# rcelha/rio-rs

Measured on NVIDIA H100. Metric: placements/sec, higher is better.
Workload: dtype u32

## Files before the change

rio_rs_b200/csrc/engine.cu:

```cuda
#include "../../include/rio_cuda.h"
#include "../../include/rio_cuda_dev.h"
#include "kernels.cuh"
#include "k_ranked.cuh"
#include "k_affinity_ranked.cuh"
#include "k_affinity_spread.cuh"
#include "k_affinity_set.cuh"
#include "k_affinity_bounded.cuh"
#include "k_set_bounded_affinity.cuh"
#include "k_set_churn.cuh"
#include "k_set_commit.cuh"
#include "k_bounded_weighted.cuh"
#include "k_changes.cuh"
#include "k_ranked_changes.cuh"
#include "k_spread.cuh"
#include "k_spread_changes.cuh"
#include "spec.cuh"
#include "trie_table.hpp"

#include <dlfcn.h>

#include <algorithm>
#include <atomic>
#include <chrono>
#include <cstdio>
// ... 231 lines not shown
    return h->h_scalars[which];
}
void check_device_error(rio_placement *h) {
    uint32_t e = 0;
    CUDA_TRY(cudaMemcpyAsync(&e, h->d_error(), 4, cudaMemcpyDeviceToHost, h->stream));
    CUDA_TRY(cudaStreamSynchronize(h->stream));
    if (e) { CUDA_TRY(cudaMemsetAsync(h->d_error(), 0, 4, h->stream)); throw RioError{RIO_ERR_UNKNOWN, "directory table overflow (internal sizing error)"}; }
}

bool address_malformed(const std::string &a) {
    size_t c = a.find(':');
    return c == std::string::npos || c == 0 || c + 1 >= a.size();
}

uint32_t intern_node(rio_placement *h, const std::string &addr) {
    auto it = h->node_index.find(addr);
    if (it != h->node_index.end()) return it->second;
    REQUIRE(h->nodes.size() < 0xFFFFFFF0u, "too many nodes");
    NodeInfo ni;
    ni.addr = addr;
    ni.seed = mix64(fnv1a64(addr.data(), addr.size()));
    ni.seed2 = mix64(ni.seed ^ kSaltNode2);
    ni.malformed = address_malformed(addr);
    uint32_t idx = (uint32_t)h->nodes.size();
    h->nodes.push_back(std::move(ni));
    h->node_index.emplace(addr, idx);
    h->tab_dirty = true;
    return idx;
}

void build_tab(rio_placement *h, TabBufs &tb, const std::vector<uint8_t> *closed) {
    const uint32_t n_total = (uint32_t)h->nodes.size();
    struct Ent { uint32_t invw, idx; };
    std::vector<Ent> live;
    auto is_closed = [&](uint32_t j) { return closed && j < closed->size() && (*closed)[j]; };
    for (uint32_t j = 0; j < n_total; j++) {
        const NodeInfo &ni = h->nodes[j];
        if (!ni.live()) continue;
        if (is_closed(j)) continue;
        live.push_back(Ent{inv_weight(ni.weight), j});
    }
    {
        std::vector<uint32_t> classes_seen;
        bool few = true;
        for (const Ent &e : live) {
            if (std::find(classes_seen.begin(), classes_seen.end(), e.invw) != classes_seen.end()) continue;
            if (classes_seen.size() == 64) { few = false; break; }
            classes_seen.push_back(e.invw);
        }
        if (few) {
            std::sort(classes_seen.begin(), classes_seen.end());
            std::vector<uint32_t> start(classes_seen.size() + 1, 0);
            auto cls = [&](uint32_t invw) { return (size_t)(std::lower_bound(classes_seen.begin(), classes_seen.end(), invw) - classes_seen.begin()); };
            for (const Ent &e : live) start[cls(e.invw) + 1]++;
            for (size_t c = 0; c < classes_seen.size(); c++) start[c + 1] += start[c];
            std::vector<Ent> grouped(live.size());
            for (const Ent &e : live) grouped[start[cls(e.invw)]++] = e;
            live.swap(grouped);
        } else {
            std::sort(live.begin(), live.end(), [](const Ent &a, const Ent &b) { return a.invw != b.invw ? a.invw < b.invw : a.idx < b.idx; });
        }
    }
    std::vector<NodeRec> recs(live.size() ? live.size() : 1);
    std::vector<ClassRec> classes;
    for (size_t q = 0; q < live.size(); q++) {
        const NodeInfo &ni = h->nodes[live[q].idx];
        recs[q] = NodeRec{(uint32_t)ni.seed, live[q].idx, (uint32_t)(ni.seed >> 32) | 1u, (uint32_t)ni.seed2};
        if (q == 0 || live[q].invw != live[q - 1].invw || (h->dev_table_flags & RIO_DEV_SPLIT_CLASSES)) classes.push_back(ClassRec{(uint32_t)q, live[q].invw});
    }
    const uint32_t n_classes = (uint32_t)classes.size();
    classes.push_back(ClassRec{(uint32_t)live.size(), 0});
    classes.push_back(ClassRec{(uint32_t)live.size(), 0});
    std::vector<uint4> by_idx(n_total ? n_total : 1);
    for (uint32_t j = 0; j < n_total; j++) {
        const NodeInfo &ni = h->nodes[j];
        const bool lv = ni.live() && !is_closed(j);
        by_idx[j] = make_uint4((uint32_t)ni.seed, lv ? inv_weight(ni.weight) : 0u, (uint32_t)(ni.seed >> 32) | 1u, (uint32_t)ni.seed2);
    }
    std::vector<TrieMember> members;
    members.reserve(live.size());
    for (const Ent &e : live) members.push_back(TrieMember{h->nodes[e.idx].seed, e.idx, h->nodes[e.idx].weight});
    const TrieBlob blob = build_trie_blob(members, h->trie_bits);
    const uint32_t bits = blob.bits, nb = 1u << bits, blob_bytes = blob.blob_bytes;
    std::vector<uint8_t> state(n_total ? n_total : 1, 0);
    std::vector<uint32_t> livef(n_total ? n_total : 1, 0);
    for (uint32_t j = 0; j < n_total; j++) {
        const NodeInfo &ni = h->nodes[j];
        state[j] = ((ni.active && !ni.malformed) ? kNodeLive : 0) | (ni.malformed ? kNodeMalformed : 0);
        livef[j] = (ni.live() && !is_closed(j)) ? 1u : 0u;
    }

    auto al = [](size_t v) { return (v + 255) & ~(size_t)255; };
    const size_t o_recs = 0, o_classes = al(o_recs + recs.size() * sizeof(NodeRec)), o_byidx = al(o_classes + classes.size() * sizeof(ClassRec)),
                 o_trie = al(o_byidx + by_idx.size() * sizeof(uint4)), o_state = al(o_trie + blob_bytes), o_live = al(o_state + state.size()),
                 total = al(o_live + livef.size() * 4);
    cudaStream_t st = h->stream;
    if (tb.upload_pending) { CUDA_TRY(cudaStreamSynchronize(st)); tb.upload_pending = false; }
    if (h->aux_stream) CUDA_TRY(cudaStreamSynchronize(h->aux_stream));
    if (total > tb.stage_cap) {
        if (tb.stage) CUDA_TRY(cudaFreeHost(tb.stage));
        tb.stage = nullptr; tb.stage_cap = 0;
        CUDA_TRY(cudaMallocHost(reinterpret_cast<void **>(&tb.stage), total * 2));
        tb.stage_cap = total * 2;
    }
    memcpy(tb.stage + o_recs, recs.data(), recs.size() * sizeof(NodeRec));
    memcpy(tb.stage + o_classes, classes.data(), classes.size() * sizeof(ClassRec));
    memcpy(tb.stage + o_byidx, by_idx.data(), by_idx.size() * sizeof(uint4));
    memcpy(tb.stage + o_trie, blob.words.data(), blob_bytes);
    memcpy(tb.stage + o_state, state.data(), state.size());
    memcpy(tb.stage + o_live, livef.data(), livef.size() * 4);
    tb.dev.ensure(total, st);
    CUDA_TRY(cudaMemcpyAsync(tb.dev.p, tb.stage, total, cudaMemcpyHostToDevice, st));
    tb.upload_pending = true;
    unsigned char *d = tb.dev.as<unsigned char>();
    tb.trie = TrieDev{d + o_trie, blob_bytes, blob.off_crec, bits, blob.n_chain, {}};
    for (uint32_t i = 1; i < 8 && i < nb; i++) tb.trie.top[i] = blob.words[i];
    tb.tab.recs = reinterpret_cast<const NodeRec *>(d + o_recs);
    tb.tab.classes = reinterpret_cast<const ClassRec *>(d + o_classes);
    tb.tab.by_idx = reinterpret_cast<const uint4 *>(d + o_byidx);
    tb.tab.n_live = (uint32_t)live.size();
    tb.tab.n_classes = n_classes;
    tb.tab.n_total = n_total;
    tb.state = d + o_state;
    tb.live = reinterpret_cast<const uint32_t *>(d + o_live);
}

uint64_t live_signature(const rio_placement *h) {
    uint64_t sig = kFnvBasis;
    for (uint32_t j = 0; j < (uint32_t)h->nodes.size(); j++)
        if (h->nodes[j].live()) sig = mix64(sig ^ (((uint64_t)j << 32) | h->nodes[j].weight));
    return sig;
}

void build_aff_operands(rio_placement *h, const std::vector<uint8_t> *closed, DevBuf &fc_buf, DevBuf &fg_buf, DevBuf &map_buf, uint32_t &n_live,
                        uint32_t &n_pad) {
    const uint32_t n_total = (uint32_t)h->nodes.size();
    cudaStream_t st = h->stream;
    auto is_closed = [&](uint32_t j) { return closed && j < closed->size() && (*closed)[j]; };
    std::vector<uint32_t> map;
    for (uint32_t j = 0; j < n_total; j++) if (h->nodes[j].live() && !is_closed(j)) map.push_back(j);
    const uint32_t nl = (uint32_t)map.size();
    const uint32_t pad = nl <= 64 ? 64 : (nl + 255) / 256 * 256;
    std::vector<float> fc((size_t)pad * 16, 0.f);
    for (uint32_t q = 0; q < nl; q++) if (h->nodes[map[q]].feat.size() == 16) std::copy(h->nodes[map[q]].feat.begin(), h->nodes[map[q]].feat.end(), fc.begin() + (size_t)q * 16);
    map.resize(pad, kNone);
    std::vector<float> fg(fc.size());
    for (uint32_t g8 = 0; g8 < pad / 8; g8++)
        for (uint32_t k4 = 0; k4 < 4; k4++)
            for (uint32_t r8 = 0; r8 < 8; r8++)
                std::copy_n(fc.begin() + ((size_t)g8 * 8 + r8) * 16 + k4 * 4, 4, fg.begin() + (((size_t)g8 * 4 + k4) * 8 + r8) * 4);
    fc_buf.ensure(fc.size() * 4, st);
    fg_buf.ensure(fg.size() * 4, st);
    CUDA_TRY(cudaMemcpyAsync(fg_buf.p, fg.data(), fg.size() * 4, cudaMemcpyHostToDevice, st));
    map_buf.ensure(map.size() * 4, st);
    CUDA_TRY(cudaMemcpyAsync(fc_buf.p, fc.data(), fc.size() * 4, cudaMemcpyHostToDevice, st));
    CUDA_TRY(cudaMemcpyAsync(map_buf.p, map.data(), map.size() * 4, cudaMemcpyHostToDevice, st));
    CUDA_TRY(cudaStreamSynchronize(st));
    n_live = nl; n_pad = pad;
}

void ensure_tab(rio_placement *h) {
    if (!h->tab_dirty) return;
    build_tab(h, h->tabs, nullptr);
    const uint32_t n_total = (uint32_t)h->nodes.size();
    cudaStream_t st = h->stream;
    h->tab_dirty = false;
    h->tab_version++;
    h->live_sig = live_signature(h);
    if (!h->K) return;
    std::vector<float> fnode((size_t)(n_total ? n_total : 1) * h->K, 0.f);
    for (uint32_t j = 0; j < n_total; j++) {
        const NodeInfo &ni = h->nodes[j];
        if (ni.feat.size() == h->K) std::copy(ni.feat.begin(), ni.feat.end(), fnode.begin() + (size_t)j * h->K);
    }
    h->d_fnode.ensure(fnode.size() * 4, st);
    CUDA_TRY(cudaMemcpyAsync(h->d_fnode.p, fnode.data(), fnode.size() * 4, cudaMemcpyHostToDevice, st));
    h->aff_live = h->aff_pad = 0;
    if (h->K == 16) build_aff_operands(h, nullptr, h->d_fnode_c, h->d_fnode_g, h->d_nidx_map, h->aff_live, h->aff_pad);
    CUDA_TRY(cudaStreamSynchronize(st));
}

uint64_t pow2_at_least(uint64_t v) { uint64_t p = 1; while (p < v) p <<= 1; return p; }

void dir_alloc(rio_placement *h, uint64_t cap, DirDev &out) {
    void *p = nullptr;
    CUDA_TRY(cudaMallocAsync(&p, cap * sizeof(DirSlot), h->stream));
    out.slots = reinterpret_cast<DirSlot *>(p);
    out.mask = cap - 1;
    uint32_t lg = 0; while ((1ull << lg) < cap) lg++;
    out.shift = 64 - lg;
    launch_dir_init(h->L(), out.slots, cap);
}

void reconcile_dir_keys(rio_placement *h) {
    h->dir_keys = read_scalar(h, S_NEWKEYS);
    h->dir_keys_pending = 0;
}

// ... 2478 lines not shown
```

rio_rs_b200/csrc/k_trie.cu:

```cuda
#include "kernels.cuh"
#include "spec.cuh"
#include "bounded_tail.cuh"

#include <cstdlib>

namespace rio {

namespace {

constexpr int kTrieThreads = 256;
constexpr uint32_t kMaxLevels = 16;

__constant__ uint32_t c_lvl_s0[kMaxLevels];
__constant__ uint32_t c_lvl_m2[kMaxLevels];
__constant__ uint32_t c_lvl_h2[kMaxLevels];

__device__ __forceinline__ uint32_t smem_u32(const void *p) { return (uint32_t)__cvta_generic_to_shared(p); }

__device__ __forceinline__ void stage_blob_tma(void *smem_dst, const void *gsrc, uint32_t bytes, unsigned long long *bar) {
    if (threadIdx.x == 0) {
        asm volatile("mbarrier.init.shared::cta.b64 [%0], 1;" ::"r"(smem_u32(bar)) : "memory");
        asm volatile("fence.mbarrier_init.release.cluster;" ::: "memory");
    }
    __syncthreads();
    if (threadIdx.x == 0) {
        asm volatile("mbarrier.arrive.expect_tx.shared::cta.b64 _, [%0], %1;" ::"r"(smem_u32(bar)), "r"(bytes) : "memory");
        for (uint32_t off = 0; off < bytes; off += 32768u) {
            const uint32_t len = min(32768u, bytes - off);
            asm volatile("cp.async.bulk.shared::cluster.global.mbarrier::complete_tx::bytes [%0], [%1], %2, [%3];"
                         ::"r"(smem_u32(reinterpret_cast<unsigned char *>(smem_dst) + off)),
                           "l"(reinterpret_cast<const unsigned char *>(gsrc) + off), "r"(len), "r"(smem_u32(bar))
                         : "memory");
        }
    }
    uint32_t done = 0;
    while (!done) {
        asm volatile("{\n\t.reg .pred p;\n\tmbarrier.try_wait.parity.shared::cta.b64 p, [%1], %2;\n\tselp.u32 %0, 1, 0, p;\n\t}"
                     : "=r"(done) : "r"(smem_u32(bar)), "r"(0u) : "memory");
    }
}

__device__ __forceinline__ uint32_t walk_step(uint32_t off, uint32_t sel) {
    uint32_t r;
    asm("mad.lo.u32 %0, %1, 2, %2;" : "=r"(r) : "r"(off), "r"(sel));
    return r;
}

template <int BITS>
__device__ __forceinline__ uint32_t trie_leaf_index(ObjHash o, const uint32_t *__restrict__ tab32, uint32_t bits_rt) {
    uint32_t i = 1;
    if (BITS > 0) {
#pragma unroll
        for (int l = 0; l < BITS; l++) {
            const uint32_t u = contest_u(o, c_lvl_s0[l], c_lvl_m2[l], c_lvl_h2[l]);
            i = 2 * i + (u > tab32[i] ? 1u : 0u);
        }
    } else {
        for (uint32_t l = 0; l < bits_rt; l++) {
            const uint32_t u = contest_u(o, c_lvl_s0[l], c_lvl_m2[l], c_lvl_h2[l]);
            i = 2 * i + (u > tab32[i] ? 1u : 0u);
        }
    }
    return i;
}

__device__ __forceinline__ uint32_t trie_resolve_leaf(ObjHash o, uint32_t leaf, const unsigned char *__restrict__ blob) {
    if ((int32_t)leaf > -2) return leaf;
    uint32_t w = leaf;
    for (;;) {
        const unsigned char *p = blob + (w & 0x7FFFFFFFu);
        const uint4 r = *reinterpret_cast<const uint4 *>(p);
        const uint2 nn = *reinterpret_cast<const uint2 *>(p + 16);
        if (contest_u(o, r.x, r.y, r.z) <= r.w) return nn.x;
        if ((int32_t)nn.y >= 0) return nn.y;
        w = nn.y;
    }
}

struct TrieSmem {
    const uint32_t *tab32;
    const unsigned char *blob;
    uint32_t *hist;
};

template <bool SMEM>
__device__ __forceinline__ TrieSmem trie_stage(const TrieDev &t, uint32_t hist_bins) {
    extern __shared__ __align__(128) unsigned char smem_trie[];
    constexpr bool in_smem = SMEM;
    TrieSmem s;
    uint32_t off = 0;
    if (in_smem) {
        s.tab32 = reinterpret_cast<const uint32_t *>(smem_trie);
        s.blob = smem_trie;
        off = t.blob_bytes;
    } else {
        const unsigned char *g = reinterpret_cast<const unsigned char *>(t.blob);
        s.tab32 = reinterpret_cast<const uint32_t *>(g);
        s.blob = g;
    }
    s.hist = reinterpret_cast<uint32_t *>(smem_trie + off);
    for (uint32_t j = threadIdx.x; j < hist_bins; j += blockDim.x) s.hist[j] = 0;
    unsigned long long *bar = reinterpret_cast<unsigned long long *>(smem_trie + off + ((hist_bins * 4u + 15u) & ~15u));
    if (in_smem) stage_blob_tma(smem_trie, t.blob, t.blob_bytes, bar);
    else __syncthreads();
    return s;
}

template <int BITS, int OPT, int MODE, bool SMEM, int MINB = (SMEM ? 5 : 3)>
__global__ void __launch_bounds__(kTrieThreads, MINB)
k_assign_trie(const uint64_t *__restrict__ keys, uint64_t n, TrieDev t, uint32_t *__restrict__ out_idx, uint32_t *__restrict__ counters,
              uint32_t hist_bins, unsigned long long *__restrict__ moved, const __grid_constant__ BoundedTail tail) {
    static_assert(OPT % 2 == 0, "two objects per 128-bit load");
    constexpr bool in_smem = SMEM;
    constexpr int SEG = OPT / 2;
    const uint64_t tile_objs = (uint64_t)kTrieThreads * OPT;
    const uint64_t n_tiles = (n + tile_objs - 1) / tile_objs;
    unsigned long long n_moved = 0;
    ulonglong2 kk[SEG];
    auto load_tile = [&](uint64_t tile) {
        const uint64_t f0 = tile * tile_objs + 2 * threadIdx.x;
        if ((tile + 1) * tile_objs <= n) {
            const ulonglong2 *src = reinterpret_cast<const ulonglong2 *>(keys + f0);
#pragma unroll
            for (int g = 0; g < SEG; g++) kk[g] = __ldg(src + g * kTrieThreads);
            return;
        }
#pragma unroll
        for (int g = 0; g < SEG; g++) {
            const uint64_t f = f0 + (uint64_t)g * (2 * kTrieThreads);
            kk[g] = make_ulonglong2(0, 0);
            if (f + 1 < n) kk[g] = __ldg(reinterpret_cast<const ulonglong2 *>(keys + f));
            else if (f < n) kk[g].x = __ldg(keys + f);
        }
    };
    const TrieSmem s = trie_stage<SMEM>(t, hist_bins);
    asm volatile("griddepcontrol.launch_dependents;" ::: "memory");
    asm volatile("griddepcontrol.wait;" ::: "memory");
    if (blockIdx.x < n_tiles) load_tile(blockIdx.x);
    for (uint64_t tile = blockIdx.x; tile < n_tiles; tile += gridDim.x) {
        const uint64_t base = tile * tile_objs;
        const bool full_tile = base + tile_objs <= n;
        ObjHash o[OPT];
#pragma unroll
        for (int g = 0; g < SEG; g++) {
            o[2 * g] = obj_hash(kk[g].x);
            o[2 * g + 1] = obj_hash(kk[g].y);
        }
        if (tile + gridDim.x < n_tiles) load_tile(tile + gridDim.x);
        uint32_t leaf[OPT];
        if (in_smem) {
            const unsigned char *tb = reinterpret_cast<const unsigned char *>(s.tab32);
            uint32_t off[OPT];
#pragma unroll
            for (int k = 0; k < OPT; k++) off[k] = 4;
            if (BITS > 0) {
                constexpr int TOP = BITS >= 3 ? 3 : 0;
                if (TOP) {
#pragma unroll
                    for (int k = 0; k < OPT; k++) {
                        const bool c0 = contest_u(o[k], c_lvl_s0[0], c_lvl_m2[0], c_lvl_h2[0]) > t.top[1];
                        const bool c1 = contest_u(o[k], c_lvl_s0[1], c_lvl_m2[1], c_lvl_h2[1]) > (c0 ? t.top[3] : t.top[2]);
                        const uint32_t t2 = c0 ? (c1 ? t.top[7] : t.top[6]) : (c1 ? t.top[5] : t.top[4]);
                        const bool c2 = contest_u(o[k], c_lvl_s0[2], c_lvl_m2[2], c_lvl_h2[2]) > t2;
                        off[k] = 32u + (c0 ? 16u : 0u) + (c1 ? 8u : 0u) + (c2 ? 4u : 0u);
                    }
                }
#pragma unroll
                for (int l = TOP; l < BITS; l++) {
#pragma unroll
                    for (int k = 0; k < OPT; k++) {
                        const uint32_t u = contest_u(o[k], c_lvl_s0[l], c_lvl_m2[l], c_lvl_h2[l]);
                        const uint32_t thr = *reinterpret_cast<const uint32_t *>(tb + off[k]);
                        off[k] = walk_step(off[k], u > thr ? 4u : 0u);
                    }
                }
            } else {
                for (uint32_t l = 0; l < t.bits; l++) {
#pragma unroll
                    for (int k = 0; k < OPT; k++) {
                        const uint32_t u = contest_u(o[k], c_lvl_s0[l], c_lvl_m2[l], c_lvl_h2[l]);
                        const uint32_t thr = *reinterpret_cast<const uint32_t *>(tb + off[k]);
                        off[k] = walk_step(off[k], u > thr ? 4u : 0u);
                    }
                }
            }
#pragma unroll
            for (int k = 0; k < OPT; k++) leaf[k] = *reinterpret_cast<const uint32_t *>(tb + off[k]);
        } else {
#pragma unroll
            for (int k = 0; k < OPT; k++) leaf[k] = __ldg(s.tab32 + trie_leaf_index<0>(o[k], s.tab32, t.bits));
        }
        uint32_t nid[OPT];
#pragma unroll
        for (int k = 0; k < OPT; k++) nid[k] = trie_resolve_leaf(o[k], leaf[k], s.blob);
        if (MODE == 0 && full_tile) {
            uint2 *dst = reinterpret_cast<uint2 *>(out_idx + base + 2 * threadIdx.x);
#pragma unroll
            for (int g = 0; g < SEG; g++) dst[g * kTrieThreads] = make_uint2(nid[2 * g], nid[2 * g + 1]);
            if (counters && nid[0] != kNone) {
                if (hist_bins) {
#pragma unroll
                    for (int k = 0; k < OPT; k++) atomicAdd(&s.hist[nid[k]], 1u);
                } else {
#pragma unroll
                    for (int k = 0; k < OPT; k++) atomicAdd(&counters[nid[k]], 1u);
                }
            }
            continue;
        }
#pragma unroll
        for (int g = 0; g < SEG; g++) {
            const uint64_t first = base + (uint64_t)g * (2 * kTrieThreads) + 2 * threadIdx.x;
            if (first >= n) continue;
            const bool two = first + 1 < n;
            if (MODE == 1) {
                uint2 old = make_uint2(kNone, kNone);
                if (two) old = *reinterpret_cast<const uint2 *>(out_idx + first);
                else old.x = out_idx[first];
                const bool c0 = old.x != nid[2 * g], c1 = two && old.y != nid[2 * g + 1];
                if (c0 | c1) {
                    if (two) *reinterpret_cast<uint2 *>(out_idx + first) = make_uint2(nid[2 * g], nid[2 * g + 1]);
                    else out_idx[first] = nid[2 * g];
                }
                n_moved += (unsigned)c0 + (unsigned)c1;
            } else {
                if (two) *reinterpret_cast<uint2 *>(out_idx + first) = make_uint2(nid[2 * g], nid[2 * g + 1]);
                else out_idx[first] = nid[2 * g];
            }
            if (counters) {
                if (hist_bins) {
                    if (nid[2 * g] != kNone) atomicAdd(&s.hist[nid[2 * g]], 1u);
                    if (two && nid[2 * g + 1] != kNone) atomicAdd(&s.hist[nid[2 * g + 1]], 1u);
                } else {
                    if (nid[2 * g] != kNone) atomicAdd(&counters[nid[2 * g]], 1u);
                    if (two && nid[2 * g + 1] != kNone) atomicAdd(&counters[nid[2 * g + 1]], 1u);
                }
            }
        }
    }
    if (MODE == 1) {
#pragma unroll
        for (int sh = 16; sh > 0; sh >>= 1) n_moved += __shfl_xor_sync(0xFFFFFFFFu, n_moved, sh);
        if ((threadIdx.x & 31) == 0 && n_moved) atomicAdd(moved, n_moved);
    }
    if (hist_bins && counters) {
        __syncthreads();
        for (uint32_t j = threadIdx.x; j < hist_bins; j += blockDim.x) { const uint32_t v = s.hist[j]; if (v) atomicAdd(&counters[j], v); }
    }
    if (MODE == 0 && tail.enabled) {
        __shared__ uint32_t s_last;
        __threadfence();
        __syncthreads();
        if (threadIdx.x == 0) s_last = atomicAdd(tail.ticket, 1u) == gridDim.x - 1;
        __syncthreads();
        if (s_last) {
            if (threadIdx.x == 0) *tail.ticket = 0;
            __threadfence();
            exchange_and_check_block(tail, counters);
        }
    }
}

template <bool SMEM>
__global__ void __launch_bounds__(kTrieThreads, 4)
k_assign_trie_sel(const uint64_t *__restrict__ keys, const uint32_t *__restrict__ sel, uint64_t n_sel, TrieDev t, uint32_t *__restrict__ out_idx,
                  uint32_t *__restrict__ counters, uint32_t hist_bins) {
    const TrieSmem s = trie_stage<SMEM>(t, hist_bins);
    for (uint64_t q = (uint64_t)blockIdx.x * blockDim.x + threadIdx.x; q < n_sel; q += (uint64_t)gridDim.x * blockDim.x) {
        const uint32_t oi = __ldg(sel + q);
        const ObjHash o = obj_hash(__ldg(keys + oi));
        const uint32_t i = trie_leaf_index<0>(o, s.tab32, t.bits);
        const uint32_t nid = trie_resolve_leaf(o, s.tab32[i], s.blob);
        out_idx[oi] = nid;
        if (counters && nid != kNone) { if (hist_bins) atomicAdd(&s.hist[nid], 1u); else atomicAdd(&counters[nid], 1u); }
    }
    if (hist_bins && counters) {
        __syncthreads();
        for (uint32_t j = threadIdx.x; j < hist_bins; j += blockDim.x) { const uint32_t v = s.hist[j]; if (v) atomicAdd(&counters[j], v); }
    }
}

template <bool SMEM>
__global__ void __launch_bounds__(kTrieThreads, 4)
k_dir_reassign_trie(DirDev dir, TrieDev t, unsigned long long *__restrict__ moved) {
    const TrieSmem s = trie_stage<SMEM>(t, 0);
    const uint4 *slots = reinterpret_cast<const uint4 *>(dir.slots);
    const uint64_t cap = dir.mask + 1;
    unsigned long long n_moved = 0;
    for (uint64_t i = (uint64_t)blockIdx.x * blockDim.x + threadIdx.x; i < cap; i += (uint64_t)gridDim.x * blockDim.x) {
        const uint4 v = slots[i];
        const unsigned long long key = ((unsigned long long)v.y << 32) | v.x;
        if (key == kEmptyKey || v.z == kNone) continue;
        const ObjHash o = obj_hash(key);
        const uint32_t li = trie_leaf_index<0>(o, s.tab32, t.bits);
        const uint32_t nid = trie_resolve_leaf(o, s.tab32[li], s.blob);
        if (nid != v.z) { reinterpret_cast<uint32_t *>(&dir.slots[i].val)[0] = nid; n_moved++; }
    }
#pragma unroll
    for (int sh = 16; sh > 0; sh >>= 1) n_moved += __shfl_xor_sync(0xFFFFFFFFu, n_moved, sh);
    if ((threadIdx.x & 31) == 0 && n_moved) atomicAdd(moved, n_moved);
}

constexpr uint32_t kTrieSmemBudget = 200u * 1024u;

struct TrieLaunchShape { uint32_t hist_bins; uint32_t in_smem; size_t smem; int ctas_per_sm; };
TrieLaunchShape trie_shape(const TrieDev &t, bool want_hist, uint32_t n_total, int want_ctas) {
    TrieLaunchShape sh{};
    sh.hist_bins = (want_hist && n_total <= 8192) ? n_total : 0;
    const size_t tail = ((size_t)sh.hist_bins * 4 + 15) / 16 * 16 + 16;
    sh.in_smem = (t.blob_bytes + tail <= kTrieSmemBudget) ? 1u : 0u;
    sh.smem = (sh.in_smem ? t.blob_bytes : 0) + tail;
    int c = want_ctas;
    while (c > 1 && (size_t)c * (sh.smem + 1024) > 227u * 1024u) c--;
    sh.ctas_per_sm = c;
    return sh;
}

bool g_lvl_uploaded[64] = {};

}

void trie_upload_level_constants(int device) {
    if (device >= 0 && device < 64 && g_lvl_uploaded[device]) return;
    uint32_t s0[kMaxLevels], m2[kMaxLevels], h2[kMaxLevels];
    for (uint32_t l = 0; l < kMaxLevels; l++) {
        const ContestRec r = contest_rec(level_seed(l));
        s0[l] = r.s0; m2[l] = r.m2; h2[l] = r.h2;
    }
    cudaMemcpyToSymbol(c_lvl_s0, s0, sizeof s0);
    cudaMemcpyToSymbol(c_lvl_m2, m2, sizeof m2);
    cudaMemcpyToSymbol(c_lvl_h2, h2, sizeof h2);
    if (device >= 0 && device < 64) g_lvl_uploaded[device] = true;
}

uint64_t trie_wave_objects(int sm_count) { return (uint64_t)sm_count * 5 * kTrieThreads * 4; }

#define RIO_TRIE_LAUNCH(KERNEL, GRID, SMEM, ...)                                                                       \
    do {                                                                                                               \
        static bool attr_set[64] = {};    \
        int dev__ = 0;                                                                                                 \
        cudaGetDevice(&dev__);                                                                                         \
        if (dev__ < 0 || dev__ >= 64 || !attr_set[dev__]) {                                                            \
            cudaFuncSetAttribute(KERNEL, cudaFuncAttributeMaxDynamicSharedMemorySize, (int)kTrieSmemBudget + 1024);    \
            if (dev__ >= 0 && dev__ < 64) attr_set[dev__] = true;                                                      \
        }                                                                                                              \
        KERNEL<<<(GRID), kTrieThreads, (SMEM), L.stream>>>(__VA_ARGS__);                                               \
    } while (0)

#define RIO_TRIE_LAUNCH_PDL(KERNEL, GRID, SMEM, ...)                                                                   \
    do {                                                                                                               \
        static bool attr_set[64] = {};                                                                                 \
        static const bool pdl = [] { const char *e = getenv("RIO_TRIE_PDL"); return !(e && e[0] == '0'); }();          \
        int dev__ = 0;                                                                                                 \
        cudaGetDevice(&dev__);                                                                                         \
        if (dev__ < 0 || dev__ >= 64 || !attr_set[dev__]) {                                                            \
            cudaFuncSetAttribute(KERNEL, cudaFuncAttributeMaxDynamicSharedMemorySize, (int)kTrieSmemBudget + 1024);    \
            if (dev__ >= 0 && dev__ < 64) attr_set[dev__] = true;                                                      \
        }                                                                                                              \
        cudaLaunchConfig_t cfg__ = {};                                                                                 \
        cfg__.gridDim = dim3((unsigned)(GRID)); cfg__.blockDim = dim3(kTrieThreads);                                   \
        cfg__.dynamicSmemBytes = (SMEM); cfg__.stream = L.stream;                                                      \
        cudaLaunchAttribute at__[1];                                                                                   \
        at__[0].id = cudaLaunchAttributeProgrammaticStreamSerialization;                                               \
        at__[0].val.programmaticStreamSerializationAllowed = 1;                                                        \
        cfg__.attrs = at__; cfg__.numAttrs = pdl ? 1 : 0;                                                              \
        cudaLaunchKernelEx(&cfg__, KERNEL, __VA_ARGS__);                                                               \
    } while (0)

void launch_assign_trie(const Launch &L, const uint64_t *d_keys, uint64_t n, const TrieDev &t, uint32_t *d_out_idx, uint32_t *d_counters,
                        const uint32_t *d_sel, uint64_t n_sel, uint32_t n_total, const BoundedTail *tail) {
    BoundedTail no_tail{};
    const BoundedTail &tl = tail ? *tail : no_tail;
    const uint64_t n_work = d_sel ? n_sel : n;
    if (!n_work) return;
    if (d_sel) {
        const TrieLaunchShape sh = trie_shape(t, d_counters != nullptr, n_total, 4);
        const uint64_t blocks = (n_work + kTrieThreads - 1) / kTrieThreads, cap = (uint64_t)L.sm_count * sh.ctas_per_sm;
        const int grid = (int)(blocks < cap ? blocks : cap);
        if (sh.in_smem) RIO_TRIE_LAUNCH(k_assign_trie_sel<true>, grid, sh.smem, d_keys, d_sel, n_work, t, d_out_idx, d_counters, sh.hist_bins);
        else RIO_TRIE_LAUNCH(k_assign_trie_sel<false>, grid, sh.smem, d_keys, d_sel, n_work, t, d_out_idx, d_counters, sh.hist_bins);
    } else {
        constexpr int OPT = 4;
#ifdef RIO_ASSIGN_TUNING
        if (const char *tn = getenv("RIO_TRIE_TUNE")) {
            const int code = atoi(tn);
            auto go = [&](auto kern, int opt, int minb) {
                const TrieLaunchShape sh2 = trie_shape(t, d_counters != nullptr, n_total, minb);
                const uint64_t tiles2 = (n_work + (uint64_t)kTrieThreads * opt - 1) / ((uint64_t)kTrieThreads * opt), cap2 = (uint64_t)L.sm_count * sh2.ctas_per_sm;
                cudaFuncSetAttribute(kern, cudaFuncAttributeMaxDynamicSharedMemorySize, (int)kTrieSmemBudget + 1024);
                kern<<<(int)(tiles2 < cap2 ? tiles2 : cap2), kTrieThreads, sh2.smem, L.stream>>>(d_keys, n_work, t, d_out_idx, d_counters, sh2.hist_bins, nullptr, tl);
            };
            bool done = true;
            switch (code) {
                case 25: go(k_assign_trie<12, 2, 0, true, 5>, 2, 5); break;
                case 28: go(k_assign_trie<12, 2, 0, true, 8>, 2, 8); break;
                case 44: go(k_assign_trie<12, 4, 0, true, 4>, 4, 4); break;
                case 45: go(k_assign_trie<12, 4, 0, true, 5>, 4, 5); break;
                case 63: go(k_assign_trie<12, 6, 0, true, 3>, 6, 3); break;
                case 64: go(k_assign_trie<12, 6, 0, true, 4>, 6, 4); break;
                case 83: go(k_assign_trie<12, 8, 0, true, 3>, 8, 3); break;
                default: done = false;
            }
            if (done && t.bits == 12) { RIO_COUNT_LAUNCH(L); return; }
        }
#endif
        const TrieLaunchShape sh = trie_shape(t, d_counters != nullptr, n_total, 5);
        uint64_t cap = (uint64_t)L.sm_count * sh.ctas_per_sm;
        if (L.spare_ctas > 0 && cap > (uint64_t)L.spare_ctas + 1) cap -= (uint64_t)L.spare_ctas;
        const uint64_t tiles = (n_work + (uint64_t)kTrieThreads * OPT - 1) / ((uint64_t)kTrieThreads * OPT);
        const int grid = (int)(tiles < cap ? tiles : cap);
        unsigned long long *no_moved = nullptr;
        if (!sh.in_smem) RIO_TRIE_LAUNCH_PDL((k_assign_trie<0, OPT, 0, false>), grid, sh.smem, d_keys, n_work, t, d_out_idx, d_counters, sh.hist_bins, no_moved, tl);
        else if (t.bits == 12) RIO_TRIE_LAUNCH_PDL((k_assign_trie<12, OPT, 0, true>), grid, sh.smem, d_keys, n_work, t, d_out_idx, d_counters, sh.hist_bins, no_moved, tl);
        else RIO_TRIE_LAUNCH_PDL((k_assign_trie<0, OPT, 0, true>), grid, sh.smem, d_keys, n_work, t, d_out_idx, d_counters, sh.hist_bins, no_moved, tl);
    }
    RIO_COUNT_LAUNCH(L);
}

void launch_reassign_trie(const Launch &L, const uint64_t *d_keys, uint64_t n, const TrieDev &t, uint32_t *d_idx, uint32_t *d_counters,
                          uint32_t n_total, unsigned long long *d_moved) {
    if (!n) return;
    constexpr int OPT = 4;
 const TrieLaunchShape sh = trie_shape(t, d_counters != nullptr, n_total, 5);
    const uint64_t tiles = (n + (uint64_t)kTrieThreads * OPT - 1) / ((uint64_t)kTrieThreads * OPT), cap = (uint64_t)L.sm_count * sh.ctas_per_sm;
    const int grid = (int)(tiles < cap ? tiles : cap);
    if (!sh.in_smem) RIO_TRIE_LAUNCH((k_assign_trie<0, OPT, 1, false>), grid, sh.smem, d_keys, n, t, d_idx, d_counters, sh.hist_bins, d_moved, BoundedTail{});
    else if (t.bits == 12) RIO_TRIE_LAUNCH((k_assign_trie<12, OPT, 1, true>), grid, sh.smem, d_keys, n, t, d_idx, d_counters, sh.hist_bins, d_moved, BoundedTail{});
    else RIO_TRIE_LAUNCH((k_assign_trie<0, OPT, 1, true>), grid, sh.smem, d_keys, n, t, d_idx, d_counters, sh.hist_bins, d_moved, BoundedTail{});
    RIO_COUNT_LAUNCH(L);
}

void launch_dir_reassign_trie(const Launch &L, const DirDev &dir, const TrieDev &t, unsigned long long *d_moved) {
    const TrieLaunchShape sh = trie_shape(t, false, 0, 4);
    const uint64_t blocks = (dir.mask + 1 + kTrieThreads - 1) / kTrieThreads, cap = (uint64_t)L.sm_count * sh.ctas_per_sm;
    const int grid = (int)(blocks < cap ? blocks : cap);
    if (sh.in_smem) RIO_TRIE_LAUNCH(k_dir_reassign_trie<true>, grid, sh.smem, dir, t, d_moved);
    else RIO_TRIE_LAUNCH(k_dir_reassign_trie<false>, grid, sh.smem, dir, t, d_moved);
    RIO_COUNT_LAUNCH(L);
}

}
```

rio_rs_b200/csrc/kernels.cuh:

```cuda
#pragma once
#include <cuda_runtime.h>
#include <cstdint>

#include "buffer_align.cuh"

namespace rio {

struct __align__(16) NodeRec {
    uint32_t s0;
    uint32_t nidx;
    uint32_t s1;
    uint32_t s2;
};
struct ClassRec {
    uint32_t start;
    uint32_t invw;
};
struct NodeTabDev {
    const NodeRec *recs;
    const ClassRec *classes;
    uint32_t n_live;
    uint32_t n_classes;
    uint32_t n_total;
    const uint4 *by_idx;
};

struct TrieDev {
    const void *blob;
    uint32_t blob_bytes;
    uint32_t off_crec;
    uint32_t bits;
    uint32_t n_chain;
    uint32_t top[8];
};

struct __align__(16) DirSlot {
    unsigned long long key;
    unsigned long long val;
};
constexpr unsigned long long kEmptyKey = 0xFFFFFFFFFFFFFFFFull;
constexpr unsigned long long kEmptyVal = 0x00000000FFFFFFFFull;
struct DirDev {
    DirSlot *slots;
    uint64_t mask;
    uint32_t shift;
};

struct Launch { cudaStream_t stream; int sm_count; uint64_t *launch_counter; int spare_ctas = 0;  };
#define RIO_COUNT_LAUNCH(L) do { if ((L).launch_counter) ++*(L).launch_counter; } while (0)

struct XchgPeers { uint32_t *win[16]; };
struct BoundedTail {
    uint32_t enabled;
    uint32_t M;
    uint32_t *ticket;
    uint32_t *next_zero;
    XchgPeers peers;
    uint32_t rank, world, max_nodes, xchg_epoch;
    uint32_t *glob;
    const uint32_t *cap;
    const uint8_t *state;
    uint32_t *closed_epoch;
    uint32_t call_epoch;
    uint32_t *thr;
    uint8_t *over;
    volatile uint32_t *host_flags;
    uint32_t flag_seq;
};

void launch_assign_hrw(const Launch &L, const uint64_t *d_keys, uint64_t n, const NodeTabDev &tab, uint32_t *d_out_idx,
                       uint32_t *d_counters , const uint32_t *d_sel , uint64_t n_sel);
uint64_t assign_wave_objects(int sm_count);
void trie_upload_level_constants(int device);
uint64_t trie_wave_objects(int sm_count);
void launch_assign_affinity(const Launch &L, const float *d_fobj, uint64_t n, const float *d_fnode ,
                            const uint32_t *d_live , uint32_t n_total, uint32_t K, uint32_t *d_out_idx,
                            float *d_out_cost , uint32_t *d_counters);
uint32_t affinity_umma_max_nodes();
void affinity_umma_set_timing_buffer(unsigned long long *d);
cudaError_t launch_assign_affinity_umma(const Launch &L, const float *d_fobj, uint64_t n, const float *d_fnode_c, const float *d_fnode_g, const uint32_t *d_nidx_map, uint32_t n_live,
                                 uint32_t m_pad, uint32_t n_total, uint32_t *d_out_idx, float *d_out_cost, uint32_t *d_counters);
uint64_t launch_mix_rate(const Launch &L, uint32_t iters, uint32_t *d_sink);
void launch_synth_keys(const Launch &L, uint64_t *d_keys, uint64_t first, uint64_t n, uint64_t seed);
void launch_hash_ids(const Launch &L, const char *d_packed, const uint64_t *d_offsets, uint64_t n, uint64_t *d_keys);
void launch_fill_u32(const Launch &L, uint32_t *d, uint64_t n, uint32_t v);
void launch_histogram(const Launch &L, const uint32_t *d_idx, uint64_t n, uint32_t *d_counters, uint32_t n_total);

void launch_select_spill(const Launch &L, const uint64_t *d_keys, const uint32_t *d_idx, uint64_t n, const uint32_t *d_thr ,
                         const uint8_t *d_over, uint32_t round, uint32_t *d_sel, unsigned long long *d_nsel, uint32_t *d_counters);

void launch_rebalance_join(const Launch &L, const uint64_t *d_keys, uint32_t *d_idx, uint64_t n, const NodeTabDev &tab, uint32_t new_idx,
                           uint32_t *d_counters, unsigned long long *d_moved);
void launch_select_on_node(const Launch &L, const uint32_t *d_idx, uint64_t n, uint32_t node, uint32_t *d_sel, unsigned long long *d_nsel);

void launch_dir_init(const Launch &L, DirSlot *slots, uint64_t cap);
void launch_dir_lookup(const Launch &L, const DirDev &dir, const uint64_t *d_keys, uint64_t n, uint32_t *d_out);
void launch_dir_upsert(const Launch &L, const DirDev &dir, const uint64_t *d_keys, const uint32_t *d_idx , uint32_t const_idx,
                       uint64_t n, uint32_t seq_base, unsigned long long *d_new_keys, uint32_t *d_error);
void launch_dir_clear_seq(const Launch &L, const DirDev &dir);
void launch_dir_clean_node(const Launch &L, const DirDev &dir, uint32_t node, unsigned long long *d_removed);
void launch_dir_clean_flagged(const Launch &L, const DirDev &dir, const uint8_t *d_flag, uint32_t n_total, unsigned long long *d_removed);
void launch_dir_rehash(const Launch &L, const DirDev &from, const DirDev &to, unsigned long long *d_new_keys, uint32_t *d_error);
void launch_dir_count(const Launch &L, const DirDev &dir, unsigned long long *d_placed, uint32_t *d_counters , uint32_t n_total);
void launch_dir_rebalance_join(const Launch &L, const DirDev &dir, const NodeTabDev &tab, uint32_t new_idx, unsigned long long *d_moved);
void launch_dir_rebalance_leave(const Launch &L, const DirDev &dir, const NodeTabDev &tab, uint32_t gone_idx, unsigned long long *d_moved);

void launch_assign_trie(const Launch &L, const uint64_t *d_keys, uint64_t n, const TrieDev &t, uint32_t *d_out_idx, uint32_t *d_counters ,
                        const uint32_t *d_sel , uint64_t n_sel, uint32_t n_total, const BoundedTail *tail = nullptr);
void launch_reassign_trie(const Launch &L, const uint64_t *d_keys, uint64_t n, const TrieDev &t, uint32_t *d_idx, uint32_t *d_counters ,
                          uint32_t n_total, unsigned long long *d_moved);
void launch_dir_reassign_trie(const Launch &L, const DirDev &dir, const TrieDev &t, unsigned long long *d_moved);

void launch_classify(const Launch &L, const uint32_t *d_cur, uint64_t n, const uint8_t *d_node_state, uint32_t n_total, uint32_t *d_sel,
                     unsigned long long *d_nsel, uint8_t *d_dead_flag);
void launch_check_address(const Launch &L, const uint32_t *d_idx, uint64_t n, const uint8_t *d_verdict_tab, uint32_t n_total, uint8_t *d_out, uint8_t *d_dead_flag,
                          unsigned long long *d_ndead);
// ... 14 lines not shown
```

rio_rs_b200/csrc/trie_table.hpp:

```cpp
#pragma once
#include <algorithm>
#include <cstdint>
#include <memory>
#include <vector>

#include "spec.cuh"

namespace rio {

struct TrieMember {
    uint64_t seed;
    uint32_t idx;
    uint32_t weight;
};

struct TrieBlob {
    std::vector<uint32_t> words;
    uint32_t blob_bytes = 0;
    uint32_t off_crec = 0;
    uint32_t n_chain = 0;
    uint32_t bits = 0;
    std::vector<uint64_t> wsum;
};

inline uint32_t contest_t3_fast(uint64_t wl, uint64_t wr) {
    if (wl == 0) return 0u;
    if (wr == 0) return 0xFFFFFFFFu;
    const uint64_t s = wl + wr;
    if (s >= (1ull << 32)) return contest_t3(wl, wr);
    const uint64_t num = wl << 31;
    uint64_t q = (uint64_t)((double)num / (double)s);
    while (q * s > num) q--;
    while ((q + 1) * s <= num) q++;
    return q ? (uint32_t)(2 * q - 1) : 0u;
}

inline TrieBlob build_trie_blob(const std::vector<TrieMember> &members, uint32_t bits) {
    const uint32_t nb = 1u << bits;
    struct Mem { uint64_t pos; uint64_t seed; uint32_t idx, w; };
    std::vector<uint32_t> bstart((size_t)nb + 1, 0);
    std::vector<Mem> all;
    all.reserve(members.size());
    for (const TrieMember &m : members) {
        if (!m.weight) continue;
        const uint64_t pos = mix64(m.seed ^ kSaltPos);
        all.push_back(Mem{pos, m.seed, m.idx, m.weight});
        bstart[(bits ? (uint32_t)(pos >> (64 - bits)) : 0u) + 1]++;
    }
    for (uint32_t k = 0; k < nb; k++) bstart[k + 1] += bstart[k];
    std::unique_ptr<Mem[]> mem(new Mem[all.size() ? all.size() : 1]);
    {
        std::vector<uint32_t> fill(bstart.begin(), bstart.end() - 1);
        for (const Mem &m : all) mem[fill[bits ? (uint32_t)(m.pos >> (64 - bits)) : 0u]++] = m;
    }
    std::vector<uint64_t> wsum((size_t)2 * nb, 0);
    uint32_t n_rec = 0;
    for (uint32_t k = 0; k < nb; k++) {
        const uint32_t lo = bstart[k], hi = bstart[k + 1];
        if (hi - lo > 1) {
            std::sort(mem.get() + lo, mem.get() + hi, [](const Mem &a, const Mem &b) { return a.pos != b.pos ? a.pos < b.pos : a.idx < b.idx; });
            n_rec += hi - lo - 1;
        }
        uint64_t sum = 0;
        for (uint32_t q = lo; q < hi; q++) sum += mem[q].w;
        wsum[nb + k] = sum;
    }
    for (uint32_t i = nb - 1; i >= 1; i--) wsum[i] = wsum[2 * i] + wsum[2 * i + 1];
    TrieBlob b;
    b.bits = bits;
    b.off_crec = (uint32_t)(((size_t)2 * nb * 4 + 15) / 16 * 16);
    b.n_chain = n_rec;
    b.blob_bytes = std::max<uint32_t>(16u, b.off_crec + n_rec * 32u);
    b.words.assign(b.blob_bytes / 4, 0u);
    uint32_t *w32 = b.words.data();
    for (uint32_t i = 1; i < nb; i++) w32[i] = contest_t3_fast(wsum[2 * i], wsum[2 * i + 1]);
    uint32_t rec_off = b.off_crec;
    for (uint32_t k = 0; k < nb; k++) {
        const uint32_t lo = bstart[k], hi = bstart[k + 1];
        if (lo == hi) { w32[nb + k] = kNone; continue; }
        if (hi - lo == 1) { w32[nb + k] = mem[lo].idx; continue; }
        w32[nb + k] = 0x80000000u | rec_off;
        uint64_t rest = wsum[nb + k];
        for (uint32_t q = lo; q + 1 < hi; q++, rec_off += 32u) {
            rest -= mem[q].w;
            const ContestRec r = contest_rec(mem[q].seed);
            uint32_t *d = w32 + rec_off / 4;
            d[0] = r.s0; d[1] = r.m2; d[2] = r.h2; d[3] = contest_t3_fast(mem[q].w, rest);
            d[4] = mem[q].idx;
            d[5] = q + 2 == hi ? mem[hi - 1].idx : 0x80000000u | (rec_off + 32u);
        }
    }
    b.wsum = std::move(wsum);
    return b;
}

inline std::vector<ContestRec> trie_level_constants(uint32_t levels) {
    std::vector<ContestRec> v(levels);
    for (uint32_t l = 0; l < levels; l++) v[l] = contest_rec(level_seed(l));
    return v;
}

inline uint32_t trie_walk_host(const uint32_t *blob, uint32_t bits, const ContestRec *level, ObjHash o) {
    uint32_t i = 1;
    for (uint32_t l = 0; l < bits; l++) i = 2 * i + (contest_u(o, level[l].s0, level[l].m2, level[l].h2) > blob[i] ? 1u : 0u);
    uint32_t w = blob[i];
    if ((int32_t)w > -2) return w;
    for (;;) {
        const uint32_t *p = blob + (w & 0x7FFFFFFFu) / 4;
        if (contest_u(o, p[0], p[1], p[2]) <= p[3]) return p[4];
        if ((int32_t)p[5] >= 0) return p[5];
        w = p[5];
    }
}

}
```

Measured before the change: 162.6 billion.

## Pack last trie level with paired 16-bit leaves into a dense shared-memory layout

Builds a second, denser trie image for 12-bit tries. Each last-level threshold is stored next to its two children's leaves, packed as 16-bit values, and chain records are rebased so they remain reachable. The walk kernel gets a PAIR variant that does the final level with one 64-bit load and a byte-permute in place of a separate leaf load, and launches with a higher CTA-per-SM target because the shared footprint is smaller. It falls back to the plain layout when leaf ids or chain indices do not fit in 15 bits, and it can be disabled with an environment variable. The change also adds a profiling script.

Result: slower. 158.9 billion, median of 6 (-2.3%).

```diff
diff --git a/_prof_tmp.py b/_prof_tmp.py
--- /dev/null
+++ b/_prof_tmp.py
@@ -0,0 +1,54 @@
+import os, sys, json, statistics
+sys.path.insert(0, os.path.dirname(os.path.abspath(__file__)))
+import torch
+from torch.profiler import profile, ProfilerActivity
+from rio_rs_b200 import build
+build.build()
+import rio_rs_b200 as R
+from oracle import pyoracle as O
+
+n, M, NS, D = 10_000_000, 1024, 4, 3
+p = R.GpuObjectPlacement(device=0)
+addrs, seeds, w = O.synth_nodes(M)
+p.set_nodes(addrs, w)
+p.set_solver("hrw2", 12)
+sets = []
+for k in range(NS):
+    s = p.new_set(n); s.synth_keys(0, n, 1 + k); sets.append(s)
+p.sync()
+
+def run(k):
+    for i in range(k):
+        sets[i % NS].assign_bounded_begin(n, 5, 4, 4)
+        if i >= D:
+            sets[(i - D) % NS].assign_bounded_end()
+    for i in range(max(0, k - D), k):
+        sets[i % NS].assign_bounded_end()
+
+import time
+for layout in ["plain", "fused", "plain", "fused"]:
+    if layout == "plain": os.environ["RIO_TRIE_LEAFPAIR"] = "0"
+    else: os.environ.pop("RIO_TRIE_LEAFPAIR", None)
+    run(50); p.sync()
+    t0 = time.perf_counter(); p.event_record(0); run(1000); p.event_record(1); p.sync(); t1 = time.perf_counter()
+    ev = p.event_elapsed_ms(0, 1)
+    with profile(activities=[ProfilerActivity.CUDA]) as prof:
+        run(200); p.sync()
+    evs = [e for e in prof.events() if e.device_type == torch.autograd.DeviceType.CUDA]
+    byname = {}
+    for e in evs:
+        byname.setdefault(e.name[:60], []).append(e)
+    walk = sorted([e for e in evs if "k_assign_trie" in e.name], key=lambda e: e.time_range.start)
+    starts = [e.time_range.start for e in walk]
+    periods = [b - a for a, b in zip(starts, starts[1:])]
+    gaps = [walk[i + 1].time_range.start - walk[i].time_range.end for i in range(len(walk) - 1)]
+    out = {"layout": layout, "step_us_events": ev, "host_us_per_step": (t1 - t0) * 1e6 / 1000,
+           "walk_us_median": statistics.median([e.time_range.elapsed_us() for e in walk]),
+           "period_us_median": statistics.median(periods), "gap_us_median": statistics.median(gaps),
+           "kernels": {k: (len(v), round(statistics.median([e.time_range.elapsed_us() for e in v]), 2)) for k, v in byname.items()}}
+    print(json.dumps(out))
+q = p.new_set(1024); q.synth_keys(0, 1024, 1); p.sync()
+t0 = time.perf_counter()
+for i in range(2000):
+    q.assign_bounded_begin(n, 5, 4, 4); q.assign_bounded_end()
+p.sync(); print("tiny set begin+end us", (time.perf_counter() - t0) * 1e6 / 2000)
diff --git a/rio_rs_b200/csrc/engine.cu b/rio_rs_b200/csrc/engine.cu
--- a/rio_rs_b200/csrc/engine.cu
+++ b/rio_rs_b200/csrc/engine.cu
@@ -337,6 +337,7 @@
     for (const Ent &e : live) members.push_back(TrieMember{h->nodes[e.idx].seed, e.idx, h->nodes[e.idx].weight});
     const TrieBlob blob = build_trie_blob(members, h->trie_bits);
     const uint32_t bits = blob.bits, nb = 1u << bits, blob_bytes = blob.blob_bytes;
+    const TrieDense dense = bits == 12 ? build_trie_dense(blob) : TrieDense{};
     std::vector<uint8_t> state(n_total ? n_total : 1, 0);
     std::vector<uint32_t> livef(n_total ? n_total : 1, 0);
     for (uint32_t j = 0; j < n_total; j++) {
@@ -347,7 +348,8 @@
 
     auto al = [](size_t v) { return (v + 255) & ~(size_t)255; };
     const size_t o_recs = 0, o_classes = al(o_recs + recs.size() * sizeof(NodeRec)), o_byidx = al(o_classes + classes.size() * sizeof(ClassRec)),
-                 o_trie = al(o_byidx + by_idx.size() * sizeof(uint4)), o_state = al(o_trie + blob_bytes), o_live = al(o_state + state.size()),
+                 o_trie = al(o_byidx + by_idx.size() * sizeof(uint4)), o_dense = al(o_trie + blob_bytes), o_state = al(o_dense + dense.bytes),
+                 o_live = al(o_state + state.size()),
                  total = al(o_live + livef.size() * 4);
     cudaStream_t st = h->stream;
     if (tb.upload_pending) { CUDA_TRY(cudaStreamSynchronize(st)); tb.upload_pending = false; }
@@ -362,13 +364,14 @@
     memcpy(tb.stage + o_classes, classes.data(), classes.size() * sizeof(ClassRec));
     memcpy(tb.stage + o_byidx, by_idx.data(), by_idx.size() * sizeof(uint4));
     memcpy(tb.stage + o_trie, blob.words.data(), blob_bytes);
+    if (dense.bytes) memcpy(tb.stage + o_dense, dense.words.data(), dense.bytes);
     memcpy(tb.stage + o_state, state.data(), state.size());
     memcpy(tb.stage + o_live, livef.data(), livef.size() * 4);
     tb.dev.ensure(total, st);
     CUDA_TRY(cudaMemcpyAsync(tb.dev.p, tb.stage, total, cudaMemcpyHostToDevice, st));
     tb.upload_pending = true;
     unsigned char *d = tb.dev.as<unsigned char>();
-    tb.trie = TrieDev{d + o_trie, blob_bytes, blob.off_crec, bits, blob.n_chain, {}};
+    tb.trie = TrieDev{d + o_trie, blob_bytes, blob.off_crec, bits, blob.n_chain, {}, d + o_dense, dense.bytes, dense.off_crec};
     for (uint32_t i = 1; i < 8 && i < nb; i++) tb.trie.top[i] = blob.words[i];
     tb.tab.recs = reinterpret_cast<const NodeRec *>(d + o_recs);
     tb.tab.classes = reinterpret_cast<const ClassRec *>(d + o_classes);
diff --git a/rio_rs_b200/csrc/k_trie.cu b/rio_rs_b200/csrc/k_trie.cu
--- a/rio_rs_b200/csrc/k_trie.cu
+++ b/rio_rs_b200/csrc/k_trie.cu
@@ -64,17 +64,30 @@
     return i;
 }
 
-__device__ __forceinline__ uint32_t trie_resolve_leaf(ObjHash o, uint32_t leaf, const unsigned char *__restrict__ blob) {
-    if ((int32_t)leaf > -2) return leaf;
-    uint32_t w = leaf;
+__device__ __forceinline__ uint32_t trie_resolve_chain(ObjHash o, const unsigned char *p, const unsigned char *__restrict__ blob) {
     for (;;) {
-        const unsigned char *p = blob + (w & 0x7FFFFFFFu);
         const uint4 r = *reinterpret_cast<const uint4 *>(p);
         const uint2 nn = *reinterpret_cast<const uint2 *>(p + 16);
         if (contest_u(o, r.x, r.y, r.z) <= r.w) return nn.x;
         if ((int32_t)nn.y >= 0) return nn.y;
-        w = nn.y;
-    }
+        p = blob + (nn.y & 0x7FFFFFFFu);
+    }
+}
+
+__device__ __forceinline__ uint32_t trie_resolve_leaf(ObjHash o, uint32_t leaf, const unsigned char *__restrict__ blob) {
+    if ((int32_t)leaf > -2) return leaf;
+    return trie_resolve_chain(o, blob + (leaf & 0x7FFFFFFFu), blob);
+}
+
+__device__ __forceinline__ uint32_t trie_pair_leaf(uint32_t u, uint2 rec) {
+    uint32_t leaf;
+    asm("prmt.b32 %0, %1, 0, %2;" : "=r"(leaf) : "r"(rec.y), "r"(u > rec.x ? 0xBB32u : 0x9910u));
+    return leaf;
+}
+
+__device__ __forceinline__ uint32_t trie_resolve_leaf16(ObjHash o, uint32_t leaf, const unsigned char *__restrict__ blob, uint32_t off_crec) {
+    if ((int32_t)leaf > -2) return leaf;
+    return trie_resolve_chain(o, blob + off_crec + ((leaf & 0x7FFFu) << 5), blob);
 }
 
 struct TrieSmem {
@@ -106,11 +119,12 @@
     return s;
 }
 
-template <int BITS, int OPT, int MODE, bool SMEM, int MINB = (SMEM ? 5 : 3)>
+template <int BITS, int OPT, int MODE, bool SMEM, int MINB = (SMEM ? 5 : 3), bool PAIR = false>
 __global__ void __launch_bounds__(kTrieThreads, MINB)
 k_assign_trie(const uint64_t *__restrict__ keys, uint64_t n, TrieDev t, uint32_t *__restrict__ out_idx, uint32_t *__restrict__ counters,
               uint32_t hist_bins, unsigned long long *__restrict__ moved, const __grid_constant__ BoundedTail tail) {
     static_assert(OPT % 2 == 0, "two objects per 128-bit load");
+    static_assert(!PAIR || (SMEM && BITS >= 3), "the dense form is walked from shared memory at a fixed depth");
     constexpr bool in_smem = SMEM;
     constexpr int SEG = OPT / 2;
     const uint64_t tile_objs = (uint64_t)kTrieThreads * OPT;
@@ -166,7 +180,7 @@
                     }
                 }
 #pragma unroll
-                for (int l = TOP; l < BITS; l++) {
+                for (int l = TOP; l < BITS - (PAIR ? 1 : 0); l++) {
 #pragma unroll
                     for (int k = 0; k < OPT; k++) {
                         const uint32_t u = contest_u(o[k], c_lvl_s0[l], c_lvl_m2[l], c_lvl_h2[l]);
@@ -174,6 +188,14 @@
                         off[k] = walk_step(off[k], u > thr ? 4u : 0u);
                     }
                 }
+                if (PAIR) {
+#pragma unroll
+                    for (int k = 0; k < OPT; k++) {
+                        const uint32_t u = contest_u(o[k], c_lvl_s0[BITS - 1], c_lvl_m2[BITS - 1], c_lvl_h2[BITS - 1]);
+                        const uint2 rec = *reinterpret_cast<const uint2 *>(tb + 2 * off[k] - (2u << BITS));
+                        leaf[k] = trie_pair_leaf(u, rec);
+                    }
+                }
             } else {
                 for (uint32_t l = 0; l < t.bits; l++) {
 #pragma unroll
@@ -184,15 +206,17 @@
                     }
                 }
             }
-#pragma unroll
-            for (int k = 0; k < OPT; k++) leaf[k] = *reinterpret_cast<const uint32_t *>(tb + off[k]);
+            if (!PAIR) {
+#pragma unroll
+                for (int k = 0; k < OPT; k++) leaf[k] = *reinterpret_cast<const uint32_t *>(tb + off[k]);
+            }
         } else {
 #pragma unroll
             for (int k = 0; k < OPT; k++) leaf[k] = __ldg(s.tab32 + trie_leaf_index<0>(o[k], s.tab32, t.bits));
         }
         uint32_t nid[OPT];
 #pragma unroll
-        for (int k = 0; k < OPT; k++) nid[k] = trie_resolve_leaf(o[k], leaf[k], s.blob);
+        for (int k = 0; k < OPT; k++) nid[k] = PAIR ? trie_resolve_leaf16(o[k], leaf[k], s.blob, t.off_crec) : trie_resolve_leaf(o[k], leaf[k], s.blob);
         if (MODE == 0 && full_tile) {
             uint2 *dst = reinterpret_cast<uint2 *>(out_idx + base + 2 * threadIdx.x);
 #pragma unroll
@@ -317,6 +341,17 @@
 }
 
 bool g_lvl_uploaded[64] = {};
+
+constexpr int kPairCtas = 6;
+
+bool trie_pair_view(TrieDev &t) {
+    const char *e = getenv("RIO_TRIE_LEAFPAIR");
+    if ((e && e[0] == '0') || t.bits != 12 || !t.dense_bytes) return false;
+    t.blob = t.dense;
+    t.blob_bytes = t.dense_bytes;
+    t.off_crec = t.dense_off_crec;
+    return true;
+}
 
 }
 
@@ -404,13 +439,17 @@
             if (done && t.bits == 12) { RIO_COUNT_LAUNCH(L); return; }
         }
 #endif
-        const TrieLaunchShape sh = trie_shape(t, d_counters != nullptr, n_total, 5);
+        TrieLaunchShape sh = trie_shape(t, d_counters != nullptr, n_total, 5);
+        TrieDev tp = t;
+        const bool pair = sh.in_smem && trie_pair_view(tp);
+        if (pair) sh = trie_shape(tp, d_counters != nullptr, n_total, kPairCtas);
         uint64_t cap = (uint64_t)L.sm_count * sh.ctas_per_sm;
         if (L.spare_ctas > 0 && cap > (uint64_t)L.spare_ctas + 1) cap -= (uint64_t)L.spare_ctas;
         const uint64_t tiles = (n_work + (uint64_t)kTrieThreads * OPT - 1) / ((uint64_t)kTrieThreads * OPT);
         const int grid = (int)(tiles < cap ? tiles : cap);
         unsigned long long *no_moved = nullptr;
         if (!sh.in_smem) RIO_TRIE_LAUNCH_PDL((k_assign_trie<0, OPT, 0, false>), grid, sh.smem, d_keys, n_work, t, d_out_idx, d_counters, sh.hist_bins, no_moved, tl);
+        else if (pair) RIO_TRIE_LAUNCH_PDL((k_assign_trie<12, OPT, 0, true, kPairCtas, true>), grid, sh.smem, d_keys, n_work, tp, d_out_idx, d_counters, sh.hist_bins, no_moved, tl);
         else if (t.bits == 12) RIO_TRIE_LAUNCH_PDL((k_assign_trie<12, OPT, 0, true>), grid, sh.smem, d_keys, n_work, t, d_out_idx, d_counters, sh.hist_bins, no_moved, tl);
         else RIO_TRIE_LAUNCH_PDL((k_assign_trie<0, OPT, 0, true>), grid, sh.smem, d_keys, n_work, t, d_out_idx, d_counters, sh.hist_bins, no_moved, tl);
     }
@@ -421,10 +460,14 @@
                           uint32_t n_total, unsigned long long *d_moved) {
     if (!n) return;
     constexpr int OPT = 4;
- const TrieLaunchShape sh = trie_shape(t, d_counters != nullptr, n_total, 5);
+    TrieLaunchShape sh = trie_shape(t, d_counters != nullptr, n_total, 5);
+    TrieDev tp = t;
+    const bool pair = sh.in_smem && trie_pair_view(tp);
+    if (pair) sh = trie_shape(tp, d_counters != nullptr, n_total, kPairCtas);
     const uint64_t tiles = (n + (uint64_t)kTrieThreads * OPT - 1) / ((uint64_t)kTrieThreads * OPT), cap = (uint64_t)L.sm_count * sh.ctas_per_sm;
     const int grid = (int)(tiles < cap ? tiles : cap);
     if (!sh.in_smem) RIO_TRIE_LAUNCH((k_assign_trie<0, OPT, 1, false>), grid, sh.smem, d_keys, n, t, d_idx, d_counters, sh.hist_bins, d_moved, BoundedTail{});
+    else if (pair) RIO_TRIE_LAUNCH((k_assign_trie<12, OPT, 1, true, kPairCtas, true>), grid, sh.smem, d_keys, n, tp, d_idx, d_counters, sh.hist_bins, d_moved, BoundedTail{});
     else if (t.bits == 12) RIO_TRIE_LAUNCH((k_assign_trie<12, OPT, 1, true>), grid, sh.smem, d_keys, n, t, d_idx, d_counters, sh.hist_bins, d_moved, BoundedTail{});
     else RIO_TRIE_LAUNCH((k_assign_trie<0, OPT, 1, true>), grid, sh.smem, d_keys, n, t, d_idx, d_counters, sh.hist_bins, d_moved, BoundedTail{});
     RIO_COUNT_LAUNCH(L);
diff --git a/rio_rs_b200/csrc/kernels.cuh b/rio_rs_b200/csrc/kernels.cuh
--- a/rio_rs_b200/csrc/kernels.cuh
+++ b/rio_rs_b200/csrc/kernels.cuh
@@ -32,6 +32,9 @@
     uint32_t bits;
     uint32_t n_chain;
     uint32_t top[8];
+    const void *dense;
+    uint32_t dense_bytes;
+    uint32_t dense_off_crec;
 };
 
 struct __align__(16) DirSlot {
diff --git a/rio_rs_b200/csrc/trie_table.hpp b/rio_rs_b200/csrc/trie_table.hpp
--- a/rio_rs_b200/csrc/trie_table.hpp
+++ b/rio_rs_b200/csrc/trie_table.hpp
@@ -100,17 +100,69 @@
     return v;
 }
 
+struct TrieDense {
+    std::vector<uint32_t> words;
+    uint32_t bytes = 0;
+    uint32_t off_crec = 0;
+};
+
+inline TrieDense build_trie_dense(const TrieBlob &b) {
+    TrieDense d;
+    if (b.bits < 3) return d;
+    const uint32_t nb = 1u << b.bits, h = nb / 2;
+    const uint32_t *w32 = b.words.data();
+    auto leaf16 = [&](uint32_t w, uint32_t &out) {
+        if (w == kNone) { out = 0xFFFFu; return true; }
+        if (!(w & 0x80000000u)) { out = w; return w <= 0x7FFFu; }
+        const uint32_t j = ((w & 0x7FFFFFFFu) - b.off_crec) / 32u;
+        out = 0x8000u | j;
+        return j < 0x7FFFu;
+    };
+    std::vector<uint32_t> words((size_t)3 * h + (size_t)b.n_chain * 8, 0u);
+    for (uint32_t i = 1; i < h; i++) words[i] = w32[i];
+    for (uint32_t i = h; i < nb; i++) {
+        uint32_t lo, hi;
+        if (!leaf16(w32[2 * i], lo) || !leaf16(w32[2 * i + 1], hi)) return d;
+        words[2 * i - h] = w32[i];
+        words[2 * i - h + 1] = lo | hi << 16;
+    }
+    d.off_crec = 12u * h;
+    for (uint32_t r = 0; r < b.n_chain; r++) {
+        const uint32_t *s = w32 + b.off_crec / 4 + 8 * r;
+        uint32_t *t = words.data() + d.off_crec / 4 + 8 * r;
+        for (int q = 0; q < 8; q++) t[q] = s[q];
+        if (t[5] & 0x80000000u) t[5] = 0x80000000u | (t[5] - 0x80000000u - b.off_crec + d.off_crec);
+    }
+    d.words = std::move(words);
+    d.bytes = (uint32_t)(d.words.size() * 4);
+    return d;
+}
+
+inline uint32_t trie_chain_host(const uint32_t *blob, const uint32_t *p, ObjHash o) {
+    for (;;) {
+        if (contest_u(o, p[0], p[1], p[2]) <= p[3]) return p[4];
+        if ((int32_t)p[5] >= 0) return p[5];
+        p = blob + (p[5] & 0x7FFFFFFFu) / 4;
+    }
+}
+
 inline uint32_t trie_walk_host(const uint32_t *blob, uint32_t bits, const ContestRec *level, ObjHash o) {
     uint32_t i = 1;
     for (uint32_t l = 0; l < bits; l++) i = 2 * i + (contest_u(o, level[l].s0, level[l].m2, level[l].h2) > blob[i] ? 1u : 0u);
-    uint32_t w = blob[i];
+    const uint32_t w = blob[i];
     if ((int32_t)w > -2) return w;
-    for (;;) {
-        const uint32_t *p = blob + (w & 0x7FFFFFFFu) / 4;
-        if (contest_u(o, p[0], p[1], p[2]) <= p[3]) return p[4];
-        if ((int32_t)p[5] >= 0) return p[5];
-        w = p[5];
-    }
+    return trie_chain_host(blob, blob + (w & 0x7FFFFFFFu) / 4, o);
+}
+
+inline uint32_t trie_walk_host_dense(const uint32_t *dense, uint32_t bits, uint32_t off_crec, const ContestRec *level, ObjHash o) {
+    uint32_t i = 1;
+    for (uint32_t l = 0; l + 1 < bits; l++) i = 2 * i + (contest_u(o, level[l].s0, level[l].m2, level[l].h2) > dense[i] ? 1u : 0u);
+    const uint32_t *r = dense + 2 * i - (1u << (bits - 1));
+    const ContestRec &c = level[bits - 1];
+    const uint32_t half = contest_u(o, c.s0, c.m2, c.h2) > r[0] ? r[1] >> 16 : r[1] & 0xFFFFu;
+    const uint32_t w = (uint32_t)(int32_t)(int16_t)half;
+    if ((int32_t)w > -2) return w;
+    return trie_chain_host(dense, dense + (off_crec + (w & 0x7FFFu) * 32u) / 4, o);
 }
 
 }
```
